# ossamaAhmed/blackbox_mpc

Hardware: AMD Instinct MI355X
Metric: MPC control-steps/sec (agent-control-steps; Pendulum true model, CEM N=500 H=30) (higher is better)
Workload: dtype f32; 1 GPU; BASELINE cfg2: Pendulum-v0 true dynamics, CEM, num_agents=1/GPU, N=500, H=30, 5 iters, k=50, closed loop (the model is the environment); parallelism=single GPU

## Files before the change

blackbox_mpc_amd/csrc/bbmpc.hip:

```cpp
#include "engine.hpp"
#include "abi_util.hpp"
#include "engine_util.hpp"
#include "kernels_corr.hpp"
#include "kernels_elite_carry.hpp"

#include <math.h>
#include <stdio.h>
#include <stdlib.h>
#include <atomic>
#include <functional>
#include <chrono>
#include <mutex>
#include <set>
#include <thread>
#include <utility>

namespace bbmpc {

static std::mutex g_engines_mu;
static std::set<Engine*> g_engines;
static std::atomic<int> g_resident_handles{0};
void note_resident_handle() { g_resident_handles.fetch_add(1, std::memory_order_relaxed); }

void stop_foreign_residents(Engine* self) {
// ... 131 lines not shown
        HIP_CHECK(hipSetDevice(c.device));
    }
    HIP_CHECK(hipGetDevice(&device));
    HIP_CHECK(hipDeviceGetAttribute(&cu_count, hipDeviceAttributeMultiprocessorCount, device));
    {
        int least = 0, greatest = 0;
        HIP_CHECK(hipDeviceGetStreamPriorityRange(&least, &greatest));
        if (!(own_stream = masked_stream_from_env("BBMPC_STREAM_CUS", cu_count)))
            HIP_CHECK(hipStreamCreateWithPriority(&own_stream, hipStreamNonBlocking, greatest));
    }
    stream = own_stream;
    init_tnq_table();

    if (const char* fm = getenv("BBMPC_FUSED")) fused_mode = atoi(fm);
    {
        auto flag = [](const char* n) { return getenv(n) != nullptr; };
        auto ival = [](const char* n, int dflt) { const char* v = getenv(n); return v ? atoi(v) : dflt; };
        sw.cma_svd_v1 = flag("BBMPC_CMA_SVD_V1"); sw.cma_svd_rounds = flag("BBMPC_CMA_SVD_ROUNDS");
        sw.cma_svd_general = flag("BBMPC_CMA_SVD_GENERAL");
        sw.cma_svd_gram = flag("BBMPC_CMA_SVD_GRAM");
        sw.cma_coop = flag("BBMPC_CMA_COOP"); sw.cma_nb = ival("BBMPC_CMA_NB", 0);
        sw.cma_eigh = ival("BBMPC_CMA_EIGH", 1); sw.cma_eigh_fail = flag("BBMPC_CMA_EIGH_FAIL");
        sw.cma_fused = flag("BBMPC_CMA_FUSED");
        sw.mlp_generic = flag("BBMPC_MLP_GENERIC");
        { const int b = ival("BBMPC_MLP_BF16", 0); sw.mlp_bf16 = (b == 1 || b == 3) ? b : 0; }
        sw.mlp_pair = ival("BBMPC_MLP_PAIR", -1); sw.mlp_q4 = ival("BBMPC_MLP_Q4", -1); sw.mlp_q4s = ival("BBMPC_MLP_Q4S", ival("BBMPC_MLP_Q4R", 1)); sw.mlp_w4 = ival("BBMPC_MLP_W4", 1); sw.pi2_skip_init = ival("BBMPC_PI2_SKIP_INIT", 1); sw.step_graph = ival("BBMPC_STEP_GRAPH", 1); sw.cma_small3 = ival("BBMPC_CMA_SMALL3", 1);
        sw.refit_wgs = ival("BBMPC_REFIT_WGS", 0);
        sw.mlp_wave = ival("BBMPC_MLP_WAVE", 1);
        sw.linger_us = std::max(0, ival("BBMPC_LINGER_US", 200));
        if (const char* fb = getenv("BBMPC_FUSED_BOUND")) {
            sw.fused_bound = atoi(fb);
            REQUIRE(sw.fused_bound == 512 || sw.fused_bound == 1024, BBMPC_E_INVALID, "BBMPC_FUSED_BOUND must be 512, 1024 or unset");
        }
        linger_test_quit = ival("BBMPC_LINGER_TEST_QUIT", 0) - 1;
        host_seq = (uint32_t)ival("BBMPC_TEST_HOST_SEQ", 0);
        sw.balance = ival("BBMPC_BALANCE", 0);
        sw.ilp = ival("BBMPC_ILP", 1) == 2 ? 2 : 1;
        sw.refit_v1 = flag("BBMPC_REFIT_V1");
        sw.zero_copy = !flag("BBMPC_NO_ZERO_COPY");
        sw.host_poll = !flag("BBMPC_NO_HOST_POLL");
        sw.mlp_no_half_tail = flag("BBMPC_MLP_NO_HALF_TAIL");
        sw.dbg = flag("BBMPC_DBG");
        sw.prof_reward_mlp = flag("BBMPC_PROF_REWARD_MLP");
        user_stepwise_only = flag("BBMPC_USER_STEPWISE");
        if (c.optimizer != BBMPC_OPT_NONE) {
            ps_loopback = auto_split > 1 ? auto_split : ival("BBMPC_POPSHARD_LOOPBACK", 0);
            ps_force = flag("BBMPC_POPSHARD_FORCE");
        }
    }
    HU = H * U;
    Nst = ((std::max(N, 1) + 63) / 64) * 64;
    rec = U + S + 1;
    lo.assign(c.action_low, c.action_low + U);
    hi.assign(c.action_high, c.action_high + U);
    upload(d_lo, lo);
    upload(d_hi, hi);
    d_state.alloc((size_t)A * S);
    d_record.alloc((size_t)A * rec);
    d_action.alloc((size_t)A * U);
    d_action.zero(stream);
    if (c.optimizer != BBMPC_OPT_NONE) {
        std::vector<float> m((size_t)A * HU), v((size_t)A * HU);
        for (int i = 0; i < A * HU; ++i) {
            const int u = i % U;
            m[i] = (lo[u] + hi[u]) / 2.0f;
            const float d = lo[u] - hi[u];
// ... 2165 lines not shown
```

blackbox_mpc_amd/csrc/bbmpc_fused.hip:

```cpp
#define BBMPC_TU_FUSED
#include "engine.hpp"
#include "engine_util.hpp"

#include <atomic>
#include <chrono>

namespace bbmpc {

void bbmpc_tu_fused_upload_tnq(const float2* table) { tnq_upload(table); }

bool Engine::use_fused() const {
    if (cfg.dynamics != BBMPC_DYN_PENDULUM || cfg.reward != BBMPC_REW_PENDULUM) return false;
    if (pop_sharded()) return false;
    if (particles_on()) return false;
    if (corr_on()) return false;
    if (carry_on()) return false;
    if (prior_on()) return false;
    if (grad_on()) return false;
    if (cfg.optimizer == BBMPC_OPT_SPSA) {
        if (iters > FUSED_MAX_SPSA_ITERS) return false;
    } else if (cfg.optimizer != BBMPC_OPT_RANDOM_SEARCH && cfg.optimizer != BBMPC_OPT_CEM && cfg.optimizer != BBMPC_OPT_PI2) {
        return false;
    }
    if (fused_mode == 0) return false;
    if (fused_mode == 1) return true;
    return (long)N <= 2048 || A >= 64;
}

static constexpr size_t fused_lds_limit() {
#ifdef BBMPC_KERNEL_DBG
    return 158 * 1024;
#else
    return 160 * 1024;
#endif
}

static void note_inst(Engine& e, int opt, bool samples_lds, bool fastm, int inj, int ilp, int maxt, bool linger) {
    snprintf(e.dominant_inst, sizeof(e.dominant_inst), "k_fused_pendulum<%d, %s, %s, %d, %d, %d, %s>", opt, samples_lds ? "true" : "false",
             fastm ? "true" : "false", inj, ilp, maxt, linger ? "true" : "false");
}

template <int OPT, int INJ, int ILP>
constexpr bool fused_has_bound512() { return OPT == FOPT_CEM && (INJ == 2 || INJ == 1) && ILP == 1; }

template <int OPT, bool FASTM, int INJ, int ILP, int MAXT>
static void launch_fused5(Engine& e, FusedArgs& fa, int threads, size_t lds_base, size_t lds_samples);

template <int OPT, bool FASTM, int INJ, int ILP>
static void launch_fused4(Engine& e, FusedArgs& fa, int threads, size_t lds_base, size_t lds_samples) {
    if constexpr (fused_has_bound512<OPT, INJ, ILP>()) {
        if (threads <= 512 && e.sw.fused_bound != 1024 && lds_base + lds_samples <= fused_lds_limit()) {
            REQUIRE(threads <= 512, BBMPC_E_HIP, "internal: a 512-bounded k_fused_pendulum launched with more threads");
            launch_fused5<OPT, FASTM, INJ, ILP, 512>(e, fa, threads, lds_base, lds_samples);
            return;
        }
    }
    REQUIRE(threads <= 1024, BBMPC_E_HIP, "internal: k_fused_pendulum launched with more than 1024 threads");
    launch_fused5<OPT, FASTM, INJ, ILP, 1024>(e, fa, threads, lds_base, lds_samples);
}

template <int OPT, bool FASTM, int INJ, int ILP, int MAXT>
static void launch_fused5(Engine& e, FusedArgs& fa, int threads, size_t lds_base, size_t lds_samples) {
    const size_t limit = fused_lds_limit();
    if (lds_base + lds_samples <= limit) {
        fa.test_quit_agent = -1;
        if constexpr (INJ == 2 && FASTM && ILP == 1) {
            if (e.linger_launch && e.subset_n == 0 && fa.done_flag && e.tail.event == nullptr) {
                auto fl = k_fused_pendulum<OPT, true, FASTM, INJ, ILP, MAXT, true>;
                note_inst(e, OPT, true, FASTM, INJ, ILP, MAXT, true);
                ensure_max_lds((const void*)fl, (int)limit);
                if (e.rec != kCompletionRecordFloats) throw HipError(BBMPC_E_HIP, "internal: the resident pendulum kernel's record is not 5 floats");
                for (int a = 0; a < e.A; ++a) {
                    volatile uint32_t* m = e.mbox_host(a);
                    volatile uint32_t* cl = e.ack_host(a);
                    for (int i = 0; i < 16; ++i) cl[i] = (fa.done_value - 1u) & 0xffffu;                    for (int i = 0; i < 13; ++i) m[i] = fa.done_value & 0xffffu;
                    m[15] = fa.done_value;
                    *(volatile uint32_t*)e.gone_host(a) = 0u;
                }
                std::atomic_thread_fence(std::memory_order_release);
                fa.done_flag = e.sync_dev(e.ack_host(0));
                fa.mbox = e.sync_dev(e.mbox_host(0));
                fa.gone = e.sync_dev(e.gone_host(0));
                fa.linger_ticks = (unsigned)e.sw.linger_us * 100u;
                fa.test_quit_agent = e.linger_test_quit;
                hipLaunchKernelGGL(fl, dim3(e.A), dim3(threads), lds_base + lds_samples, e.stream, fa);
// ... 78 lines not shown
void Engine::optimize_fused(const float* d_state_in, int add_noise, float* d_record_out, float* d_next_out, uint32_t step) {
    FusedArgs fa;
    memset(&fa, 0, sizeof(fa));
    fa.N = N; fa.A = A; fa.H = H; fa.U = U; fa.HU = HU; fa.Nst = Nst; fa.k = k; fa.iters = iters;
    fa.agent_offset = cfg.agent_offset;
    fa.fix_q1 = fix(BBMPC_FIX_Q1_REWARD_ARG_ORDER);
    fa.fix_q7 = fix(BBMPC_FIX_Q7_EXPL_NOISE_ZERO_MEAN);
    fa.add_noise = add_noise;
    fa.warm_start = fix(BBMPC_FIX_Q2_CEM_WARM_START);
    tail.publish_into(fa);
    fa.alpha = cfg.alpha;
    fa.inv_lamda = 1.0f / cfg.lamda;
    fa.state = d_state_in;
    fa.lo = d_lo.p; fa.hi = d_hi.p;
    fa.prev_mean = d_prev_mean.p; fa.var0 = d_var0.p;
    fa.mean_out = d_mean.p; fa.var_out = d_var.p;
    fa.samples_g = d_samples.p;
    fa.inj = injected(cfg.optimizer == BBMPC_OPT_RANDOM_SEARCH ? BBMPC_NOISE_UNIFORM
                      : cfg.optimizer == BBMPC_OPT_SPSA ? BBMPC_NOISE_RADEMACHER : BBMPC_NOISE_TRUNC_NORMAL);
    fa.inj_expl = injected(BBMPC_NOISE_EXPLORATION);
    if (cfg.optimizer == BBMPC_OPT_SPSA) {
        const float big_a = (float)iters / 10.0f;
        for (int it = 0; it < iters && it < FUSED_MAX_SPSA_ITERS; ++it) {
            const float tf = (float)it;
            fa.spsa_ak[it] = cfg.spsa_a / (float)pow((double)((tf + 1.0f) + big_a), (double)cfg.spsa_alpha);
            fa.spsa_ck[it] = cfg.spsa_c / (float)pow((double)(tf + 1.0f), (double)cfg.spsa_gamma);
        }
    }
    fa.record = d_record_out;
    fa.next_state = d_next_out;
    if (trace_on) {
        ensure_trace();
        fa.t_rewards = t_rewards.p; fa.t_mean = t_mean.p; fa.t_var = t_var.p; fa.t_elites = t_elites.p; fa.t_passes = t_passes.p; fa.t_samples = t_samples.p;
        if (cfg.optimizer == BBMPC_OPT_SPSA) {
            if (!t_rewards2.p) t_rewards2.alloc((size_t)A * Nst * std::max(iters, 1));
            fa.t_rewards2 = t_rewards2.p;
        }
    }
#ifdef BBMPC_KERNEL_DBG
    static long long* dbg_buf = nullptr;
    if (sw.dbg) {
        if (!dbg_buf) {
            HIP_CHECK(hipHostMalloc((void**)&dbg_buf, 64 * 8, hipHostMallocDefault));
            memset(dbg_buf, 0, 64 * 8);
        }
        if (dbg_buf[42]) {
            const long long* d = dbg_buf;
            fprintf(stderr, "[dbg] last resident pass, 10ns units rel. to its start:");
            for (int i = 0; i <= 1 + iters * 4; ++i) fprintf(stderr, " %lld", d[i] - d[0]);
            fprintf(stderr, "\n[dbg] iter0 per-wave rollout end:");
            for (int i = 24; i < 32; ++i) fprintf(stderr, " %lld", d[i] - d[0]);
            fprintf(stderr, "\n[dbg] request accepted %lld  first model step %lld  completion stored %lld\n", d[42] - d[0], d[44] - d[0], d[43] - d[0]);
            const long long sel = d[iters > 0 ? 4 * iters : 0];
            fprintf(stderr, "[dbg] tail rel. to the last selection: tail start %lld  noise applied %lld  model step %lld  record stored %lld  published %lld  last barrier %lld  carry stored %lld\n",
                    d[38] - sel, d[35] - sel, d[36] - sel, d[37] - sel, d[43] - sel, d[1 + iters * 4] - sel, d[34] - sel);
            dbg_buf[42] = 0;
        }
        fa.dbg = dbg_buf;
    }
#endif
    fa.key = key(step);
    const int pf_nit = cfg.optimizer == BBMPC_OPT_RANDOM_SEARCH ? 1 : iters;
    if (pf_mode < 0) {
        const char* ev = getenv("BBMPC_NOISE_PREFETCH");
        pf_step_floats = U == 1 ? noise_step_floats(pf_nit, A, Nst, H) : (size_t)pf_nit * A * Nst * ((HU + 3) / 4) * 4;
        const size_t budget = (size_t)128 << 20;
// ... 142 lines not shown
```

blackbox_mpc_amd/csrc/engine.hpp:

```cpp
#pragma once
#include <hip/hip_ext.h>
#include <hip/hip_runtime.h>
#include <stdint.h>
#include <string.h>

#include <algorithm>
#include <atomic>
#include <map>
#include <stdexcept>
#include <string>
#include <vector>

#include "../../include/bbmpc.h"
#include "comm.hpp"
#include "completion_line.hpp"
#include "kernels_cma.hpp"
#include "kernels_eigh.hpp"
#include "kernels_eigh_small.hpp"
#include "kernels_fused.hpp"
#include "kernels_fused_cma.hpp"
#include "kernels_fused_pso.hpp"
#include "kernels_mlp.hpp"
#include "kernels_mlp_xform.hpp"
#include "kernels_mlp_q4s.hpp"
// ... 114 lines not shown
    uint32_t step_mirror[2] = {0, 0};
    void ensure_step_words();
    bool step_capturing = false;
    int64_t calls_graph = 0;
    int64_t graph_capture_failures = 0;
    bool last_step_steady = false;
    void invalidate_step_graph() {
        ++mutations;
        step_graph_warm = 0;
        if (step_graph) { (void)hipGraphExecDestroy(step_graph); step_graph = nullptr; }
    }
    bool trace_on = false, profiling = false;
    int prof_every = 1;
    uint64_t prof_seq = 0;
    bool prof_this = false;
    int fused_mode = -1;
    struct Switches {
        bool cma_svd_v1 = false, cma_svd_rounds = false, cma_svd_general = false, cma_svd_gram = false, cma_fused = false, cma_coop = false;
        bool cma_eigh_fail = false;
        int cma_eigh = 1;
        int cma_nb = 0;
        bool mlp_generic = false;
        int mlp_bf16 = 0;
        int mlp_pair = -1, mlp_q4 = -1;
        int mlp_w4 = 1;
        int mlp_q4s = 1;
        int cma_small3 = 1;
        int step_graph = 1;
        int pi2_skip_init = 1;
        int refit_wgs = 0;
        int mlp_wave = 1;
        int linger_us = 200;
        int fused_bound = 0;
        int balance = 0;
        int ilp = 1;
        bool refit_v1 = false;
        bool zero_copy = true;
        bool mlp_no_half_tail = false;
        bool host_poll = true;
        bool prof_reward_mlp = false;
        bool dbg = false;
    } sw;

    DevBuf<float> d_lo, d_hi, d_state, d_record, d_action;
    DevBuf<float> d_prev_mean, d_var0, d_mean, d_var, d_sigma;
    DevBuf<float> d_samples, d_rewards, d_penalty;
    DevBuf<int> d_elites;
    bool mlp_ready = false;
    MlpDesc mlp;
    int mlp_nw = 1;
    DevBuf<float> d_wpack[MLP_MAX_LAYERS], d_wpack4[MLP_MAX_LAYERS], d_bpack[MLP_MAX_LAYERS], d_wraw[MLP_MAX_LAYERS], d_braw[MLP_MAX_LAYERS], d_wq4[MLP_MAX_LAYERS], d_wq4s0, d_w4pack, d_wbf[MLP_MAX_LAYERS], d_stats;
    DevBuf<float> d_fin_next, d_fin_rew, d_step_act;
    DevBuf<float> d_cand_a, d_cand_b, d_rewards2, d_vel, d_pbest, d_pbest_r, d_gbest, d_gbest_r, d_cond;
    DevBuf<int> d_gidx;
    DevBuf<float> t_rewards2;
    bool pso_seeded = false;
    int cma_G = 0, cma_n = 0;
    CmaConst cma_c;
    DevBuf<float> c_w, c_m, c_sigma, c_C, c_B, c_Dd, c_ps, c_pc, c_BD, c_z, c_Ye, c_xm, c_ym, c_evec, c_eval, c_E;
    DevBuf<int> c_eidx, c_info;
    DevBuf<unsigned> c_sync;
    DevBuf<float> e_d, e_e, e_tau, e_Vt, e_alpha, e_lam, e_Z, e_Z2, e_P, e_Tf;
    DevBuf<unsigned> e_flags;
    bool cma_use_eigh_small() const { return sw.cma_eigh && cma_n >= 2 && cma_n <= ES_N && !sw.cma_svd_v1 && !sw.cma_svd_rounds && !sw.cma_svd_general && !sw.cma_svd_gram; }
    bool cma_use_eigh() const { return sw.cma_eigh && cma_n > 128 && cma_n <= EIGH_MAX_N && (cma_n & 3) == 0 && !sw.cma_svd_v1 && !sw.cma_svd_rounds && !sw.cma_svd_general && !sw.cma_svd_gram; }
    void cma_eigh_launch(const CmaArgs& q);
// ... 357 lines not shown
```

blackbox_mpc_amd/csrc/kernels_fused.hpp:

```cpp
#pragma once
#include <type_traits>

#include "kernels_opt.hpp"
#include "kernels_refit.hpp"
#include "kernels_rollout.hpp"
#include "noise_extent.hpp"
#include "topk.hpp"

namespace bbmpc {

constexpr int FOPT_RS = 1;
constexpr int FOPT_CEM = 2;
constexpr int FOPT_PI2 = 3;
constexpr int FOPT_SPSA = 4;
constexpr int FUSED_MAX_SPSA_ITERS = 16;

struct FusedArgs {
    int N, A, H, U, HU, Nst, k, iters;
    int agent_offset;
    int fix_q1, fix_q7, add_noise;
    int warm_start;
    unsigned* done_flag;
    unsigned* done_count;
    unsigned done_value;
    float alpha, inv_lamda;
    const float* state;
    const float* lo;
    const float* hi;
    float* prev_mean;
    const float* var0;
    float* mean_out;
    float* var_out;
    float* samples_g;
    const float* inj;
    const float* inj_expl;
    float* record;
    float* next_state;
    float spsa_ak[FUSED_MAX_SPSA_ITERS], spsa_ck[FUSED_MAX_SPSA_ITERS];
    float* t_rewards2;
    float* t_rewards;
    float* t_mean;
    float* t_var;
    int* t_elites;
    float* t_samples;
    long long* dbg;
    RngKey key;
    const unsigned* mbox;
    unsigned* gone;
    unsigned linger_ticks;
    int test_quit_agent;
    const int* amap;
    const float* pf_buf[2];
    unsigned long long pf_step_floats, pf_chunk_floats;
    int* t_passes;
};


#ifdef BBMPC_KERNEL_DBG
#define BB_DBG(slot) do { if (p.dbg && tid == 0 && a == 0) dbg_lds[(slot)] = (long long)wall_clock64(); } while (0)
#else
#define BB_DBG(slot) do {} while (0)
#endif

__device__ __forceinline__ float block_min(float v, float* red, int tid, int nw) {
    v = wave_min(v);
    if ((tid & 63) == 0) red[tid >> 6] = v;
    __syncthreads();
    float r = red[(tid & 63) < nw ? (tid & 63) : 0];
    r = wave_min(r);
    __syncthreads();
    return r;
}
__device__ __forceinline__ float block_sum(float v, float* red, int tid, int nw) {
    v = wave_sum(v);
    if ((tid & 63) == 0) red[tid >> 6] = v;
    __syncthreads();
    float r = ((tid & 63) < nw) ? red[tid & 63] : 0.0f;
    r = wave_sum(r);
    __syncthreads();
    return r;
}

#ifndef BBMPC_FUSED_ACTIONS_AHEAD
#define BBMPC_FUSED_ACTIONS_AHEAD 1
#endif
#ifndef BBMPC_FUSED_EARLY_TAIL
#define BBMPC_FUSED_EARLY_TAIL 1
#endif
template <int OPT, bool SAMPLES_LDS, bool FASTM, int INJ, int ILP, int MAXT = 1024, bool LINGER = false>
__global__ __launch_bounds__(MAXT) void k_fused_pendulum(FusedArgs p) {
    static_assert(MAXT == 512 || MAXT == 1024, "k_fused_pendulum: a launch bound of 512 or 1024 threads");
    extern __shared__ __attribute__((aligned(16))) float smem[];
    const int a = p.amap ? p.amap[blockIdx.x] : (int)blockIdx.x;
    const int tid = threadIdx.x;
    const int nthr = blockDim.x;
    const int nw = nthr >> 6;
    const int HUp = (p.HU + 3) & ~3;
    const int kp = (p.k + 3) & ~3;
    float* rew = smem;
    float* mean = rew + p.Nst;
    float* var = mean + HUp;
    float* sigma = var + HUp;
    int* eidx = (int*)(sigma + HUp);
    float* red = (float*)(eidx + kp);
    uint32_t* hist = (uint32_t*)(red + 64);
    unsigned long long* ekeys = (unsigned long long*)(hist + (OPT == FOPT_CEM ? TOPK_HIST_WORDS : TOPK_HIST_WORDS_NARROW));
    float* samp = SAMPLES_LDS ? (float*)(ekeys + kp) : (p.samples_g + (size_t)a * p.HU * p.Nst);
#ifdef BBMPC_KERNEL_DBG
    __shared__ long long dbg_lds[48];
#endif
    const PendulumModel model{p.fix_q1 != 0};
    const float lo = p.lo[0], hi = p.hi[0];
    RngKey key_s = p.key;
    const float* inj_s = p.inj;
    int add_noise_s = p.add_noise;
    unsigned done_value_s = p.done_value;
    if (tid < 3) red[60 + tid] = p.state[a * 3 + tid];
    const bool keep_init = LINGER && OPT != FOPT_RS && p.HU <= nthr;
    [[maybe_unused]] float m_keep = 0.0f, v_keep = 0.0f, s_keep = 0.0f;
    auto dist_init = [&](bool from_keep) {
        if (from_keep) {
            if (tid < p.HU) {
                mean[tid] = m_keep;
                var[tid] = v_keep;
                sigma[tid] = (OPT == FOPT_CEM && p.warm_start) ? cem_sigma(m_keep, v_keep, lo, hi) : s_keep;
            }
        } else {
            for (int j = tid; j < p.HU; j += nthr) {
                const float m = p.prev_mean[a * p.HU + j];
                const float v = p.var0[a * p.HU + j];
                const float sg = (OPT == FOPT_CEM) ? cem_sigma(m, v, lo, hi) : ((OPT == FOPT_SPSA) ? 0.0f : sqrtf(v));
                mean[j] = m;
                var[j] = v;
                sigma[j] = sg;
                if (keep_init) { m_keep = m; v_keep = v; s_keep = sg; }
            }
        }
    };
    typedef float pfvec4 __attribute__((ext_vector_type(4)));
    typedef const __attribute__((address_space(1))) pfvec4* pfvec4p;
// ... 285 lines not shown
                for (int q = 0; q < ILP; ++q) gen(q, 0);
                for (int b = 0; b < nblk; ++b) {
                    float xc[ILP][4];
#pragma unroll
                    for (int q = 0; q < ILP; ++q) {
#pragma unroll
                        for (int i = 0; i < 4; ++i) xc[q][i] = xn[q][i];
                        gen(q, b + 1);
                    }
#pragma unroll
                    for (int i = 0; i < 4; ++i)
#pragma unroll
                        for (int q = 0; q < ILP; ++q) consume(q, 4 * b + i, xc[q][i]);
                }
                for (int i = 0; i < rem; ++i)
#pragma unroll
                    for (int q = 0; q < ILP; ++q) consume(q, 4 * nblk + i, xn[q][i]);
#pragma unroll
                for (int q = 0; q < ILP; ++q) {
                    float tot = roll[q].total();
                    if (tot != tot) tot = -1.0e6f;
                    if (OPT == FOPT_PI2) {
                        const float nr = sqrtf(pen[q]);
                        tot = tot - nr * nr;
                    }
                    if (live[q]) rew[nn[q]] = tot;
                }
            }
            });
#ifdef BBMPC_KERNEL_DBG
            if (p.dbg && a == 0 && it == 0 && (tid & 63) == 0) dbg_lds[24 + (tid >> 6) % 8] = (long long)wall_clock64();
#endif
            if (it + 1 < p.iters) prefetch_first(inj_s, it + 1);
            if (OPT == FOPT_CEM) block_topk_prepass(rew, p.N, p.k, hist, tid, nthr);
            BB_DBG(2 + it * 4);
            __syncthreads();
            BB_DBG(3 + it * 4);
            if (p.t_rewards) {
                if (OPT != FOPT_SPSA)
                    for (int n = tid; n < p.N; n += nthr) p.t_rewards[((size_t)it * p.A + a) * p.Nst + n] = rew[n];
                for (int i = tid; i < p.HU * p.Nst; i += nthr) {
                    const int j = i / p.Nst, n = i % p.Nst;
                    if (n < p.N) p.t_samples[(((size_t)it * p.A + a) * p.HU + j) * p.Nst + n] = samp[(size_t)j * p.Nst + n];
                }
            }

            if (OPT == FOPT_CEM) {
                const TopkSel sel = block_topk_select(rew, p.N, p.k, hist, tid, nthr, true);
                if (p.t_passes && tid == 0) p.t_passes[(size_t)it * p.A + a] = sel.passes;
                if (p.t_elites) {
                    block_topk_finish_sorted(rew, p.N, p.k, eidx, hist, ekeys, sel, tid, nthr);
                    for (int e = tid; e < p.k; e += nthr) p.t_elites[((size_t)it * p.A + a) * p.k + e] = eidx[e];
                    __syncthreads();
                }
                block_topk_finish_indexed(rew, p.N, p.k, eidx, hist, sel, tid, nthr);
                BB_DBG(4 + it * 4);
#ifdef BBMPC_KERNEL_DBG
                if (p.dbg && tid == 0 && a == 0 && it == 1) for (int i = 0; i < 12; ++i) p.dbg[48 + i] = g_topk_dbg[i];
#endif
                const float kf = (float)p.k;
                const int sub = tid & 15;
                constexpr int EC = 4;
                const bool small_k = p.k <= 16 * EC;
                int ei[EC];
#pragma unroll
                for (int i = 0; i < EC; ++i) ei[i] = (small_k && sub + 16 * i < p.k) ? eidx[sub + 16 * i] : -1;
                [[maybe_unused]] float mean_row0 = 0.0f;
                for (int j = tid >> 4; j < ((p.HU + 3) & ~3); j += nthr >> 4) {
                    const bool live = j < p.HU;
                    const float* row = samp + (size_t)(live ? j : 0) * p.Nst;
                    float sum = 0.0f, vs = 0.0f, em;
                    if (small_k) {
                        float x[EC];
#pragma unroll
                        for (int i = 0; i < EC; ++i) x[i] = row[ei[i] >= 0 ? ei[i] : 0];
#pragma unroll
                        for (int i = 0; i < EC; ++i) if (ei[i] >= 0) sum += x[i];
                        sum = row16_sum(sum);
                        em = sum / kf;
#pragma unroll
                        for (int i = 0; i < EC; ++i)
                            if (ei[i] >= 0) {
                                const float d = x[i] - em;
                                vs += d * d;
                            }
                    } else {
                        for (int e = sub; e < p.k; e += 16) sum += row[eidx[e]];
                        sum = row16_sum(sum);
// ... 169 lines not shown
```

blackbox_mpc_amd/csrc/topk.hpp:

```cpp
#pragma once
#include <hip/hip_runtime.h>
#include <stdint.h>

#include "topk_digits.hpp"

namespace bbmpc {

__device__ __forceinline__ uint32_t wave_incl_scan(uint32_t v, int lane) {
    int x = (int)v;
    x += __builtin_amdgcn_update_dpp(0, x, 0x111, 0xf, 0xf, false);
    x += __builtin_amdgcn_update_dpp(0, x, 0x112, 0xf, 0xf, false);
    x += __builtin_amdgcn_update_dpp(0, x, 0x114, 0xf, 0xf, false);
    x += __builtin_amdgcn_update_dpp(0, x, 0x118, 0xf, 0xf, false);
    const int t0 = __builtin_amdgcn_readlane(x, 15), t1 = __builtin_amdgcn_readlane(x, 31),
              t2 = __builtin_amdgcn_readlane(x, 47);
    const int row = lane >> 4;
    x += (row >= 1 ? t0 : 0) + (row >= 2 ? t1 : 0) + (row >= 3 ? t2 : 0);
    return (uint32_t)x;
}

#ifdef BBMPC_KERNEL_DBG
__shared__ long long g_topk_dbg[16];
#define TOPK_DBG(i) do { if (tid == 0) g_topk_dbg[(i)] = (long long)wall_clock64(); } while (0)
#else
#define TOPK_DBG(i) do {} while (0)
#endif

struct TopkSel {
    uint32_t kmin;
    uint32_t T;
    uint32_t lim;
    uint32_t remaining;
    uint32_t eq_total;
    int passes;
};

template <bool WIDE = true>
__device__ __forceinline__ void block_topk_prepass(const float* vals, int N, int k, uint32_t* hist, int tid, int nthr) {
    const int lane = tid & 63, wave = tid >> 6;
    uint32_t* hist2 = hist + TOPK_HIST2_OFF;
    uint32_t k1 = 0xFFFFFFFFu, kmaxl = 0u;
    for (int n = tid; n < N; n += nthr) {
        const uint32_t key = reward_key(vals[n]);
        k1 = min(k1, key);
        kmaxl = max(kmaxl, key);
    }
    uint32_t k2 = 0xFFFFFFFFu;
#define BB_ROW_MIN2(ctrl) do {                                                                              \
        const uint32_t o1 = (uint32_t)__builtin_amdgcn_update_dpp(0, (int)k1, ctrl, 0xf, 0xf, false);             \
        const uint32_t o2 = (uint32_t)__builtin_amdgcn_update_dpp(0, (int)k2, ctrl, 0xf, 0xf, false);             \
        const uint32_t hi1 = max(k1, o1);                                                                         \
        k1 = min(k1, o1);                                                                                         \
        k2 = min(hi1, min(k2, o2));                                                                               \
    } while (0)
    BB_ROW_MIN2(0xB1); BB_ROW_MIN2(0x4E); BB_ROW_MIN2(0x141); BB_ROW_MIN2(0x140);
#undef BB_ROW_MIN2
#define BB_ROW_U32(op, v, ctrl) v = op(v, (uint32_t)__builtin_amdgcn_update_dpp(0, (int)(v), ctrl, 0xf, 0xf, false))
    BB_ROW_U32(max, kmaxl, 0xB1); BB_ROW_U32(max, kmaxl, 0x4E); BB_ROW_U32(max, kmaxl, 0x141); BB_ROW_U32(max, kmaxl, 0x140);
#undef BB_ROW_U32
    const int first_round = min(N, nthr);
    const int rows_ok = first_round >= 2 ? min(nthr >> 4, ((first_round - 2) >> 4) + 1) : 0;
    const bool bound_ok = 2 * rows_ok >= k;
    uint32_t kmin = 0xFFFFFFFFu, kmax = 0u;
#pragma unroll
    for (int r = 0; r < 4; ++r) {
        const int row = wave * 4 + r;
        kmin = min(kmin, (uint32_t)__builtin_amdgcn_readlane((int)k1, 16 * r));
        const uint32_t b = bound_ok ? (uint32_t)__builtin_amdgcn_readlane((int)k2, 16 * r)
                                    : (uint32_t)__builtin_amdgcn_readlane((int)kmaxl, 16 * r);
        if (!bound_ok || row < rows_ok) kmax = max(kmax, b);
    }
    if (lane == 0) { hist2[wave] = kmin; hist2[16 + wave] = kmax; }
    uint2* hz = reinterpret_cast<uint2*>(hist + TOPK_HIST1_OFF);
    for (int i = tid; i < (WIDE ? TOPK_BINS1 : TOPK_BINSN) / 2; i += nthr) hz[i] = make_uint2(0u, 0u);
}

__device__ __forceinline__ void topk_scan_first(const uint32_t* h, uint32_t* ctrl, uint32_t remaining, int lane) {
    const uint4* hv = reinterpret_cast<const uint4*>(h);
    const uint4 c0 = hv[lane], c1 = hv[64 + lane], c2 = hv[128 + lane], c3 = hv[192 + lane];
    const uint32_t s0 = c0.x + c0.y + c0.z + c0.w, s1 = c1.x + c1.y + c1.z + c1.w;
    const uint32_t s2 = c2.x + c2.y + c2.z + c2.w, s3 = c3.x + c3.y + c3.z + c3.w;
    const uint32_t s = (s0 + s1) + (s2 + s3);
    const uint32_t incl = wave_incl_scan(s, lane);
    const uint32_t excl = incl - s;
    if (excl < remaining && remaining <= incl) {
        const uint32_t p1 = excl + s0, p2 = p1 + s1, p3 = p2 + s2;
        const bool g1 = remaining > p1, g2 = remaining > p2, g3 = remaining > p3;
        const uint32_t q = (uint32_t)g1 + (uint32_t)g2 + (uint32_t)g3;
        const uint32_t pq = g3 ? p3 : (g2 ? p2 : (g1 ? p1 : excl));
        const uint32_t x = g3 ? c3.x : (g2 ? c2.x : (g1 ? c1.x : c0.x));
        const uint32_t y = g3 ? c3.y : (g2 ? c2.y : (g1 ? c1.y : c0.y));
        const uint32_t z = g3 ? c3.z : (g2 ? c2.z : (g1 ? c1.z : c0.z));
        const uint32_t w = g3 ? c3.w : (g2 ? c2.w : (g1 ? c1.w : c0.w));
        const uint32_t e1 = pq + x, e2 = e1 + y, e3 = e2 + z;
        const bool h1 = remaining > e1, h2 = remaining > e2, h3 = remaining > e3;
        const uint32_t e = (uint32_t)h1 + (uint32_t)h2 + (uint32_t)h3;
        const uint32_t cum = h3 ? e3 : (h2 ? e2 : (h1 ? e1 : pq));
        const uint32_t cnt = h3 ? w : (h2 ? z : (h1 ? y : x));
        ctrl[0] = 16u * (uint32_t)lane + 4u * q + e;
        ctrl[1] = remaining - cum;
        ctrl[2] = cnt;
        ctrl[3] = 0;
    }
}

template <bool WIDE = true>
__device__ __forceinline__ TopkSel block_topk_select(const float* vals, int N, int k, uint32_t* hist, int tid, int nthr,
                                                     bool prepass_done = false) {
    const int lane = tid & 63, nw = nthr >> 6;
    TOPK_DBG(0);
    uint32_t* ctrl = hist + TOPK_CTRL_OFF;
    uint32_t* hist2 = hist + TOPK_HIST2_OFF;
    uint32_t* hist1 = hist + TOPK_HIST1_OFF;
    constexpr int W1 = WIDE ? TOPK_W1 : TOPK_WN;
    if (!prepass_done) {
        block_topk_prepass<WIDE>(vals, N, k, hist, tid, nthr);
        __syncthreads();
    }
    uint32_t kmin, kmax;
    TOPK_DBG(1);
    kmin = 0xFFFFFFFFu; kmax = 0u;
    if (lane < nw) { kmin = hist2[lane]; kmax = hist2[16 + lane]; }
#define BB_ROW_U32(op, v, ctrl) v = op(v, (uint32_t)__builtin_amdgcn_update_dpp(0, (int)(v), ctrl, 0xf, 0xf, false))
    BB_ROW_U32(min, kmin, 0xB1); BB_ROW_U32(min, kmin, 0x4E); BB_ROW_U32(min, kmin, 0x141); BB_ROW_U32(min, kmin, 0x140);
    BB_ROW_U32(max, kmax, 0xB1); BB_ROW_U32(max, kmax, 0x4E); BB_ROW_U32(max, kmax, 0x141); BB_ROW_U32(max, kmax, 0x140);
#undef BB_ROW_U32
    kmin = (uint32_t)__builtin_amdgcn_readlane((int)kmin, 0);
    kmax = (uint32_t)__builtin_amdgcn_readlane((int)kmax, 0);
    const TopkRange rg = topk_range(kmin, kmax);
    const uint32_t span = rg.span;
    int top = rg.top;
    uint32_t T = 0u;
    uint32_t remaining = (uint32_t)k;
    uint32_t eq_total = (uint32_t)N;
    int pass = 0;
    while (top > 0) {
        uint32_t* h = (pass & 1) ? hist2 : hist1;
        uint32_t* hn = (pass & 1) ? hist1 : hist2;
        const int shift = topk_pass_shift(pass, top, W1);
        for (int n = tid; n < N; n += nthr) {
            const uint32_t kp = topk_offset_key(vals[n], kmin);
            if (topk_takes_part(kp, span, T, top)) {
                const uint32_t d = topk_digit(kp, pass, top, W1);
                const uint32_t slot = (WIDE && pass == 0) ? topk_first_slot(d) : d;
#ifdef BBMPC_EXP_NOATOMIC
                h[slot] = 1u;
#else
                atomicAdd(&h[slot], 1u);
#endif
            }
        }
        __syncthreads();
        TOPK_DBG(2 + 2 * pass);
        if (tid < 64) {
            if (WIDE && pass == 0) {
                topk_scan_first(h, ctrl, remaining, lane);
            } else {
                const uint4 c = *reinterpret_cast<const uint4*>(h + 4 * lane);
                const uint32_t s = c.x + c.y + c.z + c.w;
                const uint32_t incl = wave_incl_scan(s, lane);
                const uint32_t excl = incl - s;
                if (excl < remaining && remaining <= incl) {
                    uint32_t cum = excl, b = 4 * lane, cnt = c.x;
                    if (cum + c.x < remaining) { cum += c.x; b += 1; cnt = c.y;
                        if (cum + c.y < remaining) { cum += c.y; b += 1; cnt = c.z;
                            if (cum + c.z < remaining) { cum += c.z; b += 1; cnt = c.w; } } }
                    ctrl[0] = b;
                    ctrl[1] = remaining - cum;
                    ctrl[2] = cnt;
                    ctrl[3] = 0;
                }
            }
        } else {
            for (int i = tid - 64; i < TOPK_BINSN; i += nthr - 64) hn[i] = 0;
        }
        if (nthr == 64)
            for (int i = tid; i < TOPK_BINSN; i += 64) hn[i] = 0;
        __syncthreads();
        TOPK_DBG(3 + 2 * pass);
        T |= (uint32_t)__builtin_amdgcn_readfirstlane((int)ctrl[0]) << shift;
        remaining = (uint32_t)__builtin_amdgcn_readfirstlane((int)ctrl[1]);
        eq_total = (uint32_t)__builtin_amdgcn_readfirstlane((int)ctrl[2]);
        top = shift;
        ++pass;
        if (eq_total == remaining) break;
    }
    if (pass == 0) {
        if (tid == 0) ctrl[3] = 0;
        __syncthreads();
        eq_total = remaining + 1u;
    }
    return TopkSel{kmin, T, topk_winner_limit(span, T, top), remaining, eq_total, pass};
}

__device__ __forceinline__ bool topk_is_winner(const float* vals, int n, const TopkSel& s) {
    const uint32_t kp = topk_offset_key(vals[n], s.kmin);
    if (s.eq_total == s.remaining) return kp <= s.lim;
    if (kp < s.T) return true;
    if (kp != s.T) return false;
    uint32_t before = 0;
    for (int m = 0; m < n; ++m) before += (topk_offset_key(vals[m], s.kmin) == s.T) ? 1u : 0u;
    return before < s.remaining;
}

__device__ __forceinline__ void block_topk_finish_indexed(const float* vals, int N, int k, int* eidx, uint32_t* hist,
                                                          const TopkSel& sel, int tid, int nthr) {
    const int lane = tid & 63, wave = tid >> 6, nw = nthr >> 6;
    uint32_t* wtot = hist;
    uint32_t base = 0;
    int round = 0;
    for (int n0 = 0; n0 < N; n0 += nthr, ++round) {
        const int n = n0 + tid;
        const bool take = (n < N) && topk_is_winner(vals, n, sel);
        const unsigned long long bal = __ballot(take);
        const uint32_t pre = __builtin_amdgcn_mbcnt_hi((uint32_t)(bal >> 32), __builtin_amdgcn_mbcnt_lo((uint32_t)bal, 0u));
        uint32_t* wt = wtot + (round & 1) * 16;
        if (lane == 0) wt[wave] = (uint32_t)__popcll(bal);
        __syncthreads();
        int x = (lane < nw) ? (int)wt[lane] : 0;
        x += __builtin_amdgcn_update_dpp(0, x, 0x111, 0xf, 0xf, false);
        x += __builtin_amdgcn_update_dpp(0, x, 0x112, 0xf, 0xf, false);
        x += __builtin_amdgcn_update_dpp(0, x, 0x114, 0xf, 0xf, false);
        x += __builtin_amdgcn_update_dpp(0, x, 0x118, 0xf, 0xf, false);
        const uint32_t tot = (uint32_t)__builtin_amdgcn_readlane(x, 15);
        const uint32_t incl_w = (uint32_t)__builtin_amdgcn_readlane(x, __builtin_amdgcn_readfirstlane(wave));
        const uint32_t off = base + incl_w - (uint32_t)__popcll(bal);
        if (take) eidx[off + pre] = n;
        base += tot;
    }
    __syncthreads();
}

__device__ __forceinline__ void block_topk_finish_sorted(const float* vals, int N, int k, int* eidx, uint32_t* hist,
                                                         unsigned long long* ekeys, const TopkSel& sel, int tid, int nthr) {
    uint32_t* ctrl = hist + TOPK_CTRL_OFF;
    const uint32_t T = sel.T, remaining = sel.remaining, eq_total = sel.eq_total, kmin = sel.kmin;
    for (int e = tid; e < k; e += nthr) eidx[e] = 0;
    if (eq_total == remaining) {
        for (int n = tid; n < N; n += nthr) {
            const uint32_t key = topk_offset_key(vals[n], kmin);
            if (key <= sel.lim) {
                const uint32_t slot = atomicAdd(&ctrl[3], 1u);
                ekeys[slot] = ((unsigned long long)key << 32) | (uint32_t)n;
            }
        }
        __syncthreads();
    } else {
        const int lane = tid & 63, wave = tid >> 6, nw = nthr >> 6;
        uint32_t* wtot = hist;
        uint32_t base = 0;
        int round = 0;
        for (int n0 = 0; n0 < N; n0 += nthr, ++round) {
            const int n = n0 + tid;
            const uint32_t key = n < N ? topk_offset_key(vals[n], kmin) : 0xFFFFFFFFu;
            const bool tie = n < N && key == T;
            const unsigned long long bal = __ballot(tie);
            const uint32_t pre = __builtin_amdgcn_mbcnt_hi((uint32_t)(bal >> 32), __builtin_amdgcn_mbcnt_lo((uint32_t)bal, 0u));
            uint32_t* wt = wtot + (round & 1) * 16;
            if (lane == 0) wt[wave] = (uint32_t)__popcll(bal);
            __syncthreads();
            uint32_t ahead = base, tot = 0;
            for (int w = 0; w < nw; ++w) { const uint32_t c = wt[w]; ahead += (w < wave) ? c : 0u; tot += c; }
            const bool take = n < N && (key < T || (tie && ahead + pre < remaining));
// ... 40 lines not shown
```

blackbox_mpc_amd/csrc/topk_digits.hpp:

```cpp
#pragma once
#include <stdint.h>
#include <string.h>

#if defined(__HIPCC__) || defined(__CUDACC__)
#define BBMPC_TOPK_HD __host__ __device__ __forceinline__
#else
#define BBMPC_TOPK_HD inline
#endif

namespace bbmpc {

constexpr int TOPK_W1 = 10;
constexpr int TOPK_WN = 8;
constexpr int TOPK_BINS1 = 1 << TOPK_W1;
constexpr int TOPK_BINSN = 1 << TOPK_WN;
constexpr int TOPK_HIST2_OFF = 0;
constexpr int TOPK_CTRL_OFF = TOPK_BINSN;
constexpr int TOPK_HIST1_OFF = TOPK_BINSN + 16;
constexpr int TOPK_HIST_WORDS = TOPK_BINSN + 16 + TOPK_BINS1;
constexpr int TOPK_HIST_WORDS_NARROW = TOPK_BINSN + 16 + TOPK_BINSN;
constexpr int TOPK_MAX_PASSES = 1 + (32 - TOPK_W1 + TOPK_WN - 1) / TOPK_WN;
static_assert(TOPK_W1 >= TOPK_WN && TOPK_W1 <= 10, "wave 0 scans the first histogram with 16 bins per lane at most");

BBMPC_TOPK_HD uint32_t reward_key(float r) {
// ... 20 lines not shown
    uint32_t kmin;
    uint32_t span;
    int top;
};
BBMPC_TOPK_HD TopkRange topk_range(uint32_t kmin, uint32_t bound) {
    const uint32_t span = bound - kmin;
    return TopkRange{kmin, span, topk_bit_length(span)};
}

BBMPC_TOPK_HD uint32_t topk_offset_key(float r, uint32_t kmin) { return reward_key(r) - kmin; }

BBMPC_TOPK_HD int topk_pass_width(int pass, int top, int w1 = TOPK_W1) {
    const int w = pass == 0 ? w1 : TOPK_WN;
    return top < w ? top : w;
}
BBMPC_TOPK_HD int topk_pass_shift(int pass, int top, int w1 = TOPK_W1) { return top - topk_pass_width(pass, top, w1); }

BBMPC_TOPK_HD uint32_t topk_digit(uint32_t kp, int pass, int top, int w1 = TOPK_W1) {
    const int w = topk_pass_width(pass, top, w1);
    return (kp >> (top - w)) & ((1u << w) - 1u);
}

BBMPC_TOPK_HD bool topk_takes_part(uint32_t kp, uint32_t span, uint32_t T, int top) {
    return kp <= span && (top >= 32 || (kp >> top) == (T >> top));
}

BBMPC_TOPK_HD uint32_t topk_first_slot(uint32_t d) { return ((d >> 2) & 3u) * 256u + ((d >> 4) << 2) + (d & 3u); }

BBMPC_TOPK_HD uint32_t topk_winner_limit(uint32_t span, uint32_t T, int top) {
    const uint32_t hi = top >= 32 ? 0xFFFFFFFFu : (T | ((1u << top) - 1u));
    return hi < span ? hi : span;
}

}
```

Before: 34650 control-steps/s.

## Add single-pass wave-level CEM top-k select with direct elite list output

Adds a specialized CEM elite-selection route for the 512-thread fused pendulum kernel. When N fits in one block and k≤64, it builds the first radix histogram with one element per thread, scans all 1024 bins in a single wave, and writes the elite index list by ballot compaction when the chosen bucket is fully taken. This avoids the multi-pass select plus the separate indexed finish step. When the bucket is split it falls back to the existing passes. The prepass also writes its min/max into separate slots and clears the second histogram early, which costs a little extra LDS work.

```diff
diff --git a/blackbox_mpc_amd/csrc/bbmpc.hip b/blackbox_mpc_amd/csrc/bbmpc.hip
--- a/blackbox_mpc_amd/csrc/bbmpc.hip
+++ b/blackbox_mpc_amd/csrc/bbmpc.hip
@@ -187,6 +187,8 @@
             sw.fused_bound = atoi(fb);
             REQUIRE(sw.fused_bound == 512 || sw.fused_bound == 1024, BBMPC_E_INVALID, "BBMPC_FUSED_BOUND must be 512, 1024 or unset");
         }
+        sw.cem_wave_select = ival("BBMPC_CEM_WAVE_SELECT", 1) != 0 ? 1 : 0;
+        sw.trace_select_only = flag("BBMPC_TRACE_SELECT_ONLY");
         linger_test_quit = ival("BBMPC_LINGER_TEST_QUIT", 0) - 1;
         host_seq = (uint32_t)ival("BBMPC_TEST_HOST_SEQ", 0);
         sw.balance = ival("BBMPC_BALANCE", 0);
diff --git a/blackbox_mpc_amd/csrc/bbmpc_fused.hip b/blackbox_mpc_amd/csrc/bbmpc_fused.hip
--- a/blackbox_mpc_amd/csrc/bbmpc_fused.hip
+++ b/blackbox_mpc_amd/csrc/bbmpc_fused.hip
@@ -51,6 +51,7 @@
     if constexpr (fused_has_bound512<OPT, INJ, ILP>()) {
         if (threads <= 512 && e.sw.fused_bound != 1024 && lds_base + lds_samples <= fused_lds_limit()) {
             REQUIRE(threads <= 512, BBMPC_E_HIP, "internal: a 512-bounded k_fused_pendulum launched with more threads");
+            fa.wave_select = (BBMPC_CEM_WAVE_SELECT && e.sw.cem_wave_select) ? 1 : 0;
             launch_fused5<OPT, FASTM, INJ, ILP, 512>(e, fa, threads, lds_base, lds_samples);
             return;
         }
@@ -195,6 +196,7 @@
     if (trace_on) {
         ensure_trace();
         fa.t_rewards = t_rewards.p; fa.t_mean = t_mean.p; fa.t_var = t_var.p; fa.t_elites = t_elites.p; fa.t_passes = t_passes.p; fa.t_samples = t_samples.p;
+        if (sw.trace_select_only) fa.t_elites = nullptr;
         if (cfg.optimizer == BBMPC_OPT_SPSA) {
             if (!t_rewards2.p) t_rewards2.alloc((size_t)A * Nst * std::max(iters, 1));
             fa.t_rewards2 = t_rewards2.p;
diff --git a/blackbox_mpc_amd/csrc/engine.hpp b/blackbox_mpc_amd/csrc/engine.hpp
--- a/blackbox_mpc_amd/csrc/engine.hpp
+++ b/blackbox_mpc_amd/csrc/engine.hpp
@@ -170,6 +170,8 @@
         int mlp_wave = 1;
         int linger_us = 200;
         int fused_bound = 0;
+        int cem_wave_select = 1;
+        bool trace_select_only = false;
         int balance = 0;
         int ilp = 1;
         bool refit_v1 = false;
diff --git a/blackbox_mpc_amd/csrc/kernels_fused.hpp b/blackbox_mpc_amd/csrc/kernels_fused.hpp
--- a/blackbox_mpc_amd/csrc/kernels_fused.hpp
+++ b/blackbox_mpc_amd/csrc/kernels_fused.hpp
@@ -53,6 +53,7 @@
     const float* pf_buf[2];
     unsigned long long pf_step_floats, pf_chunk_floats;
     int* t_passes;
+    int wave_select;
 };
 
 
@@ -81,6 +82,9 @@
     return r;
 }
 
+#ifndef BBMPC_CEM_WAVE_SELECT
+#define BBMPC_CEM_WAVE_SELECT 1
+#endif
 #ifndef BBMPC_FUSED_ACTIONS_AHEAD
 #define BBMPC_FUSED_ACTIONS_AHEAD 1
 #endif
@@ -106,6 +110,9 @@
     uint32_t* hist = (uint32_t*)(red + 64);
     unsigned long long* ekeys = (unsigned long long*)(hist + (OPT == FOPT_CEM ? TOPK_HIST_WORDS : TOPK_HIST_WORDS_NARROW));
     float* samp = SAMPLES_LDS ? (float*)(ekeys + kp) : (p.samples_g + (size_t)a * p.HU * p.Nst);
+    constexpr bool WAVE_SEL = BBMPC_CEM_WAVE_SELECT && OPT == FOPT_CEM && MAXT == 512 && SAMPLES_LDS;
+    [[maybe_unused]] uint32_t* const slot_min = (uint32_t*)red;
+    [[maybe_unused]] uint32_t* const slot_bound = (uint32_t*)red + 32;
 #ifdef BBMPC_KERNEL_DBG
     __shared__ long long dbg_lds[48];
 #endif
@@ -457,7 +464,8 @@
             if (p.dbg && a == 0 && it == 0 && (tid & 63) == 0) dbg_lds[24 + (tid >> 6) % 8] = (long long)wall_clock64();
 #endif
             if (it + 1 < p.iters) prefetch_first(inj_s, it + 1);
-            if (OPT == FOPT_CEM) block_topk_prepass(rew, p.N, p.k, hist, tid, nthr);
+            if constexpr (WAVE_SEL) block_topk_prepass<true, true>(rew, p.N, p.k, hist, tid, nthr, slot_min, slot_bound);
+            else if (OPT == FOPT_CEM) block_topk_prepass(rew, p.N, p.k, hist, tid, nthr);
             BB_DBG(2 + it * 4);
             __syncthreads();
             BB_DBG(3 + it * 4);
@@ -471,14 +479,25 @@
             }
 
             if (OPT == FOPT_CEM) {
-                const TopkSel sel = block_topk_select(rew, p.N, p.k, hist, tid, nthr, true);
-                if (p.t_passes && tid == 0) p.t_passes[(size_t)it * p.A + a] = sel.passes;
-                if (p.t_elites) {
-                    block_topk_finish_sorted(rew, p.N, p.k, eidx, hist, ekeys, sel, tid, nthr);
-                    for (int e = tid; e < p.k; e += nthr) p.t_elites[((size_t)it * p.A + a) * p.k + e] = eidx[e];
-                    __syncthreads();
-                }
-                block_topk_finish_indexed(rew, p.N, p.k, eidx, hist, sel, tid, nthr);
+                TopkSel sel;
+                [[maybe_unused]] int route = TOPK_ROUTE_OLD;
+                if constexpr (WAVE_SEL) {
+                    if (p.wave_select && p.t_elites == nullptr && p.N <= nthr && p.k <= 64)
+                        route = block_topk_wave_select(rew, p.N, p.k, eidx, hist, slot_min, slot_bound, tid, nthr, sel);
+                    else
+                        sel = block_topk_select(rew, p.N, p.k, hist, tid, nthr, true, slot_min, slot_bound);
+                } else {
+                    sel = block_topk_select(rew, p.N, p.k, hist, tid, nthr, true);
+                }
+                if (p.t_passes && tid == 0) p.t_passes[(size_t)it * p.A + a] = sel.passes | (route != TOPK_ROUTE_OLD ? 0x100 : 0);
+                if (route == TOPK_ROUTE_OLD) {
+                    if (p.t_elites) {
+                        block_topk_finish_sorted(rew, p.N, p.k, eidx, hist, ekeys, sel, tid, nthr);
+                        for (int e = tid; e < p.k; e += nthr) p.t_elites[((size_t)it * p.A + a) * p.k + e] = eidx[e];
+                        __syncthreads();
+                    }
+                    block_topk_finish_indexed(rew, p.N, p.k, eidx, hist, sel, tid, nthr);
+                }
                 BB_DBG(4 + it * 4);
 #ifdef BBMPC_KERNEL_DBG
                 if (p.dbg && tid == 0 && a == 0 && it == 1) for (int i = 0; i < 12; ++i) p.dbg[48 + i] = g_topk_dbg[i];
diff --git a/blackbox_mpc_amd/csrc/topk.hpp b/blackbox_mpc_amd/csrc/topk.hpp
--- a/blackbox_mpc_amd/csrc/topk.hpp
+++ b/blackbox_mpc_amd/csrc/topk.hpp
@@ -35,8 +35,9 @@
     int passes;
 };
 
-template <bool WIDE = true>
-__device__ __forceinline__ void block_topk_prepass(const float* vals, int N, int k, uint32_t* hist, int tid, int nthr) {
+template <bool WIDE = true, bool SPLIT = false>
+__device__ __forceinline__ void block_topk_prepass(const float* vals, int N, int k, uint32_t* hist, int tid, int nthr,
+                                                   uint32_t* smin = nullptr, uint32_t* sbound = nullptr) {
     const int lane = tid & 63, wave = tid >> 6;
     uint32_t* hist2 = hist + TOPK_HIST2_OFF;
     uint32_t k1 = 0xFFFFFFFFu, kmaxl = 0u;
@@ -70,7 +71,14 @@
                                     : (uint32_t)__builtin_amdgcn_readlane((int)kmaxl, 16 * r);
         if (!bound_ok || row < rows_ok) kmax = max(kmax, b);
     }
-    if (lane == 0) { hist2[wave] = kmin; hist2[16 + wave] = kmax; }
+    if constexpr (SPLIT) {
+        if (lane == 0) { smin[wave] = kmin; sbound[wave] = kmax; }
+        uint2* hz2 = reinterpret_cast<uint2*>(hist2);
+        for (int i = tid; i < TOPK_BINSN / 2; i += nthr) hz2[i] = make_uint2(0u, 0u);
+        if (tid == 0) hist[TOPK_CTRL_OFF + 3] = 0u;
+    } else {
+        if (lane == 0) { hist2[wave] = kmin; hist2[16 + wave] = kmax; }
+    }
     uint2* hz = reinterpret_cast<uint2*>(hist + TOPK_HIST1_OFF);
     for (int i = tid; i < (WIDE ? TOPK_BINS1 : TOPK_BINSN) / 2; i += nthr) hz[i] = make_uint2(0u, 0u);
 }
@@ -105,35 +113,14 @@
 }
 
 template <bool WIDE = true>
-__device__ __forceinline__ TopkSel block_topk_select(const float* vals, int N, int k, uint32_t* hist, int tid, int nthr,
-                                                     bool prepass_done = false) {
-    const int lane = tid & 63, nw = nthr >> 6;
-    TOPK_DBG(0);
+__device__ __forceinline__ TopkSel topk_select_passes(const float* vals, int N, uint32_t* hist, int tid, int nthr, uint32_t kmin,
+                                                      uint32_t span, int top, uint32_t T, uint32_t remaining, uint32_t eq_total,
+                                                      int pass) {
+    const int lane = tid & 63;
     uint32_t* ctrl = hist + TOPK_CTRL_OFF;
     uint32_t* hist2 = hist + TOPK_HIST2_OFF;
     uint32_t* hist1 = hist + TOPK_HIST1_OFF;
     constexpr int W1 = WIDE ? TOPK_W1 : TOPK_WN;
-    if (!prepass_done) {
-        block_topk_prepass<WIDE>(vals, N, k, hist, tid, nthr);
-        __syncthreads();
-    }
-    uint32_t kmin, kmax;
-    TOPK_DBG(1);
-    kmin = 0xFFFFFFFFu; kmax = 0u;
-    if (lane < nw) { kmin = hist2[lane]; kmax = hist2[16 + lane]; }
-#define BB_ROW_U32(op, v, ctrl) v = op(v, (uint32_t)__builtin_amdgcn_update_dpp(0, (int)(v), ctrl, 0xf, 0xf, false))
-    BB_ROW_U32(min, kmin, 0xB1); BB_ROW_U32(min, kmin, 0x4E); BB_ROW_U32(min, kmin, 0x141); BB_ROW_U32(min, kmin, 0x140);
-    BB_ROW_U32(max, kmax, 0xB1); BB_ROW_U32(max, kmax, 0x4E); BB_ROW_U32(max, kmax, 0x141); BB_ROW_U32(max, kmax, 0x140);
-#undef BB_ROW_U32
-    kmin = (uint32_t)__builtin_amdgcn_readlane((int)kmin, 0);
-    kmax = (uint32_t)__builtin_amdgcn_readlane((int)kmax, 0);
-    const TopkRange rg = topk_range(kmin, kmax);
-    const uint32_t span = rg.span;
-    int top = rg.top;
-    uint32_t T = 0u;
-    uint32_t remaining = (uint32_t)k;
-    uint32_t eq_total = (uint32_t)N;
-    int pass = 0;
     while (top > 0) {
         uint32_t* h = (pass & 1) ? hist2 : hist1;
         uint32_t* hn = (pass & 1) ? hist1 : hist2;
@@ -193,6 +180,31 @@
     return TopkSel{kmin, T, topk_winner_limit(span, T, top), remaining, eq_total, pass};
 }
 
+template <bool WIDE = true>
+__device__ __forceinline__ TopkSel block_topk_select(const float* vals, int N, int k, uint32_t* hist, int tid, int nthr,
+                                                     bool prepass_done = false, const uint32_t* smin = nullptr,
+                                                     const uint32_t* sbound = nullptr) {
+    const int lane = tid & 63, nw = nthr >> 6;
+    TOPK_DBG(0);
+    uint32_t* hist2 = hist + TOPK_HIST2_OFF;
+    if (!prepass_done) {
+        block_topk_prepass<WIDE>(vals, N, k, hist, tid, nthr);
+        __syncthreads();
+    }
+    uint32_t kmin, kmax;
+    TOPK_DBG(1);
+    kmin = 0xFFFFFFFFu; kmax = 0u;
+    if (lane < nw) { kmin = smin ? smin[lane] : hist2[lane]; kmax = sbound ? sbound[lane] : hist2[16 + lane]; }
+#define BB_ROW_U32(op, v, ctrl) v = op(v, (uint32_t)__builtin_amdgcn_update_dpp(0, (int)(v), ctrl, 0xf, 0xf, false))
+    BB_ROW_U32(min, kmin, 0xB1); BB_ROW_U32(min, kmin, 0x4E); BB_ROW_U32(min, kmin, 0x141); BB_ROW_U32(min, kmin, 0x140);
+    BB_ROW_U32(max, kmax, 0xB1); BB_ROW_U32(max, kmax, 0x4E); BB_ROW_U32(max, kmax, 0x141); BB_ROW_U32(max, kmax, 0x140);
+#undef BB_ROW_U32
+    kmin = (uint32_t)__builtin_amdgcn_readlane((int)kmin, 0);
+    kmax = (uint32_t)__builtin_amdgcn_readlane((int)kmax, 0);
+    const TopkRange rg = topk_range(kmin, kmax);
+    return topk_select_passes<WIDE>(vals, N, hist, tid, nthr, kmin, rg.span, rg.top, 0u, (uint32_t)k, (uint32_t)N, 0);
+}
+
 __device__ __forceinline__ bool topk_is_winner(const float* vals, int n, const TopkSel& s) {
     const uint32_t kp = topk_offset_key(vals[n], s.kmin);
     if (s.eq_total == s.remaining) return kp <= s.lim;
@@ -217,6 +229,7 @@
         uint32_t* wt = wtot + (round & 1) * 16;
         if (lane == 0) wt[wave] = (uint32_t)__popcll(bal);
         __syncthreads();
+        TOPK_DBG(8);
         int x = (lane < nw) ? (int)wt[lane] : 0;
         x += __builtin_amdgcn_update_dpp(0, x, 0x111, 0xf, 0xf, false);
         x += __builtin_amdgcn_update_dpp(0, x, 0x112, 0xf, 0xf, false);
@@ -229,6 +242,83 @@
         base += tot;
     }
     __syncthreads();
+    TOPK_DBG(9);
+}
+
+constexpr int TOPK_ROUTE_OLD = 0, TOPK_ROUTE_LIST = 1;
+
+struct TopkWavePick {
+    uint32_t bucket, wanted, cnt;
+};
+__device__ __forceinline__ TopkWavePick topk_scan_first_all(const uint32_t* h, uint32_t remaining, int lane) {
+    const uint4* hv = reinterpret_cast<const uint4*>(h);
+    const uint4 c0 = hv[lane], c1 = hv[64 + lane], c2 = hv[128 + lane], c3 = hv[192 + lane];
+    const uint32_t s0 = c0.x + c0.y + c0.z + c0.w, s1 = c1.x + c1.y + c1.z + c1.w;
+    const uint32_t s2 = c2.x + c2.y + c2.z + c2.w, s3 = c3.x + c3.y + c3.z + c3.w;
+    const uint32_t s = (s0 + s1) + (s2 + s3);
+    const uint32_t incl = wave_incl_scan(s, lane);
+    const uint32_t excl = incl - s;
+    const TopkPick pk = topk_pick16(TopkQuad{c0.x, c0.y, c0.z, c0.w}, TopkQuad{c1.x, c1.y, c1.z, c1.w}, TopkQuad{c2.x, c2.y, c2.z, c2.w},
+                                    TopkQuad{c3.x, c3.y, c3.z, c3.w}, excl, remaining);
+    const unsigned long long holder = __ballot(excl < remaining && remaining <= incl);
+    const int src = holder ? __builtin_ctzll(holder) : 0;
+    TopkWavePick r;
+    r.bucket = 16u * (uint32_t)src + (uint32_t)__builtin_amdgcn_readlane((int)pk.sub, src);
+    r.wanted = (uint32_t)__builtin_amdgcn_readlane((int)pk.wanted, src);
+    r.cnt = (uint32_t)__builtin_amdgcn_readlane((int)pk.cnt, src);
+    return r;
+}
+
+__device__ __forceinline__ int block_topk_wave_select(const float* vals, int N, int k, int* eidx, uint32_t* hist, const uint32_t* smin,
+                                                      const uint32_t* sbound, int tid, int nthr, TopkSel& sel) {
+    const int lane = tid & 63, wave = tid >> 6, nw = nthr >> 6;
+    uint32_t* hist1 = hist + TOPK_HIST1_OFF;
+    uint32_t kmin = 0xFFFFFFFFu, kmax = 0u;
+    if (lane < nw) { kmin = smin[lane]; kmax = sbound[lane]; }
+#define BB_ROW_U32(op, v, ctrl) v = op(v, (uint32_t)__builtin_amdgcn_update_dpp(0, (int)(v), ctrl, 0xf, 0xf, false))
+    BB_ROW_U32(min, kmin, 0xB1); BB_ROW_U32(min, kmin, 0x4E); BB_ROW_U32(min, kmin, 0x141); BB_ROW_U32(min, kmin, 0x140);
+    BB_ROW_U32(max, kmax, 0xB1); BB_ROW_U32(max, kmax, 0x4E); BB_ROW_U32(max, kmax, 0x141); BB_ROW_U32(max, kmax, 0x140);
+#undef BB_ROW_U32
+    kmin = (uint32_t)__builtin_amdgcn_readlane((int)kmin, 0);
+    kmax = (uint32_t)__builtin_amdgcn_readlane((int)kmax, 0);
+    const TopkRange rg = topk_range(kmin, kmax);
+    const uint32_t span = rg.span;
+    if (rg.top == 0) {
+        sel = topk_select_passes<true>(vals, N, hist, tid, nthr, kmin, span, 0, 0u, (uint32_t)k, (uint32_t)N, 0);
+        return TOPK_ROUTE_OLD;
+    }
+    const int shift = topk_pass_shift(0, rg.top, TOPK_W1);
+    uint32_t kp = 0xFFFFFFFFu;
+    if (tid < N) {
+        kp = topk_offset_key(vals[tid], kmin);
+        if (topk_takes_part(kp, span, 0u, rg.top)) atomicAdd(&hist1[topk_first_slot(topk_digit(kp, 0, rg.top, TOPK_W1))], 1u);
+    }
+    __syncthreads();
+    TOPK_DBG(2);
+    const TopkWavePick pk = topk_scan_first_all(hist1, (uint32_t)k, lane);
+    const uint32_t T = pk.bucket << shift;
+    if (!topk_whole_bucket_in(pk.wanted, pk.cnt)) {
+        sel = topk_select_passes<true>(vals, N, hist, tid, nthr, kmin, span, shift, T, pk.wanted, pk.cnt, 1);
+        return TOPK_ROUTE_OLD;
+    }
+    const uint32_t lim = topk_winner_limit(span, T, shift);
+    sel = TopkSel{kmin, T, lim, pk.wanted, pk.cnt, 1};
+    uint32_t* wt = hist;
+    const bool take = tid < N && kp <= lim;
+    const unsigned long long bal = __ballot(take);
+    const uint32_t pre = __builtin_amdgcn_mbcnt_hi((uint32_t)(bal >> 32), __builtin_amdgcn_mbcnt_lo((uint32_t)bal, 0u));
+    if (lane == 0) wt[wave] = (uint32_t)__popcll(bal);
+    __syncthreads();
+    TOPK_DBG(3);
+    int x = (lane < nw) ? (int)wt[lane] : 0;
+    x += __builtin_amdgcn_update_dpp(0, x, 0x111, 0xf, 0xf, false);
+    x += __builtin_amdgcn_update_dpp(0, x, 0x112, 0xf, 0xf, false);
+    x += __builtin_amdgcn_update_dpp(0, x, 0x114, 0xf, 0xf, false);
+    x += __builtin_amdgcn_update_dpp(0, x, 0x118, 0xf, 0xf, false);
+    const uint32_t incl_w = (uint32_t)__builtin_amdgcn_readlane(x, __builtin_amdgcn_readfirstlane(wave));
+    if (take) eidx[incl_w - (uint32_t)__popcll(bal) + pre] = tid;
+    __syncthreads();
+    return TOPK_ROUTE_LIST;
 }
 
 __device__ __forceinline__ void block_topk_finish_sorted(const float* vals, int N, int k, int* eidx, uint32_t* hist,
diff --git a/blackbox_mpc_amd/csrc/topk_digits.hpp b/blackbox_mpc_amd/csrc/topk_digits.hpp
--- a/blackbox_mpc_amd/csrc/topk_digits.hpp
+++ b/blackbox_mpc_amd/csrc/topk_digits.hpp
@@ -76,4 +76,32 @@
     return hi < span ? hi : span;
 }
 
+struct TopkQuad {
+    uint32_t x, y, z, w;
+};
+struct TopkPick {
+    uint32_t sub;
+    uint32_t wanted;
+    uint32_t cnt;
+};
+BBMPC_TOPK_HD TopkPick topk_pick16(TopkQuad c0, TopkQuad c1, TopkQuad c2, TopkQuad c3, uint32_t excl, uint32_t remaining) {
+    const uint32_t s0 = c0.x + c0.y + c0.z + c0.w, s1 = c1.x + c1.y + c1.z + c1.w, s2 = c2.x + c2.y + c2.z + c2.w;
+    const uint32_t p1 = excl + s0, p2 = p1 + s1, p3 = p2 + s2;
+    const bool g1 = remaining > p1, g2 = remaining > p2, g3 = remaining > p3;
+    const uint32_t q = (uint32_t)g1 + (uint32_t)g2 + (uint32_t)g3;
+    const uint32_t pq = g3 ? p3 : (g2 ? p2 : (g1 ? p1 : excl));
+    const uint32_t x = g3 ? c3.x : (g2 ? c2.x : (g1 ? c1.x : c0.x));
+    const uint32_t y = g3 ? c3.y : (g2 ? c2.y : (g1 ? c1.y : c0.y));
+    const uint32_t z = g3 ? c3.z : (g2 ? c2.z : (g1 ? c1.z : c0.z));
+    const uint32_t w = g3 ? c3.w : (g2 ? c2.w : (g1 ? c1.w : c0.w));
+    const uint32_t e1 = pq + x, e2 = e1 + y, e3 = e2 + z;
+    const bool h1 = remaining > e1, h2 = remaining > e2, h3 = remaining > e3;
+    const uint32_t e = (uint32_t)h1 + (uint32_t)h2 + (uint32_t)h3;
+    const uint32_t cum = h3 ? e3 : (h2 ? e2 : (h1 ? e1 : pq));
+    const uint32_t cnt = h3 ? w : (h2 ? z : (h1 ? y : x));
+    return TopkPick{4u * q + e, remaining - cum, cnt};
 }
+
+BBMPC_TOPK_HD bool topk_whole_bucket_in(uint32_t wanted, uint32_t cnt) { return wanted == cnt; }
+
+}
```

New measurement: 35700 control-steps/s (median of 6 runs). +3.0%, better.
